# AnnSeidel/genometools

Measured on AMD Instinct MI355X. Metric: Gbp/s ESA build (suf+lcp+bwt), 3 Gbp DNA, 1/2/4/8 MI355X; bit-exact vs CPU, higher is better.
Workload: dtype u64; 1 GPU; human-like DNA (2% N, 24 seqs, repeats) n=3000000000 seed=43 -suf -lcp -bwt (BASELINE.json configs[2]); parallelism=1 device, pair_suffixes=341032298, tied_suffixes=390540711, refine_rounds=9, maxbranchdepth=8256

## Files before the change

genometools_amd/_lib.py:

```python
import ctypes
import os
import subprocess

HERE = os.path.dirname(os.path.abspath(__file__))
ROOT = os.path.dirname(HERE)
LIB_PATH = os.path.join(HERE, "libgtamd_esa.so")
SOURCES = [os.path.join(HERE, "csrc", f) for f in
           ("esa_prims.hip", "esa_engine.hip", "esa_synth.hip", "esa_encode.hip",
            "esa_pck.hip", "esa_comm.hip")]
HEADERS = [os.path.join(HERE, "csrc", f) for f in ("esa_common.h", "esa_prims.h", "esa_devutil.h", "esa_msd.h", "esa_msd_blocks.h",
                                                     "esa_pck_replay.h")] + \
          [os.path.join(ROOT, "include", h) for h in ("gtamd_esa.h", "gtamd_encode.h", "gtamd_pck.h")]
HIPCC = os.environ.get("HIPCC", "/opt/rocm/bin/hipcc")


def needs_build():
    if not os.path.exists(LIB_PATH):
        return True
    t = os.path.getmtime(LIB_PATH)
    return any(os.path.getmtime(p) > t for p in SOURCES + HEADERS)


def build_library(force=False, verbose=False):
    if not force and not needs_build():
        return LIB_PATH
    cmd = [HIPCC, "--offload-arch=gfx950", "-O3", "-std=c++17", "-fPIC",
           "-shared", "-Wall", "-Wno-unused-function", "-o", LIB_PATH] + SOURCES
    if verbose:
        print(" ".join(cmd))
    subprocess.run(cmd, check=True)
    return LIB_PATH


class EsaStats(ctypes.Structure):
    _fields_ = [("totallength", ctypes.c_uint64),
                ("numberofallsortedsuffixes", ctypes.c_uint64),
                ("longest", ctypes.c_uint64),
                ("largelcpvalues", ctypes.c_uint64),
                ("maxbranchdepth", ctypes.c_uint64),
                ("lcptabsum", ctypes.c_uint64),
                ("prefixlength", ctypes.c_uint32),
                ("refine_rounds", ctypes.c_uint32),
                ("tied_suffixes", ctypes.c_uint64),
                ("pair_suffixes", ctypes.c_uint64),
                ("device_bytes", ctypes.c_uint64),
                ("msd_big_entries", ctypes.c_uint64),
                ("msd_crowded_entries", ctypes.c_uint64),
                ("rank_entries_built", ctypes.c_uint64)]


class EsaTiming(ctypes.Structure):
    _fields_ = [("total_ms", ctypes.c_float),
                ("keygen_ms", ctypes.c_float),
                ("sort_ms", ctypes.c_float),
                ("finalize_ms", ctypes.c_float),
                ("refine_ms", ctypes.c_float),
                ("tie_fix_ms", ctypes.c_float),
                ("scatter_ms", ctypes.c_float),
                ("scatter_launches", ctypes.c_uint32),
                ("scatter_items", ctypes.c_uint64),
                ("comm_ms", ctypes.c_float),
                ("comm_calls", ctypes.c_uint32),
                ("comm_bytes", ctypes.c_uint64),
                ("alloc_ms", ctypes.c_float),
                ("dominant_kernel", ctypes.c_uint32),
                ("scatter_read_items", ctypes.c_uint64),
                ("scatter_written_items", ctypes.c_uint64)]


class EncodeSummary(ctypes.Structure):
    _fields_ = [(name, ctypes.c_uint64) for name in
                ("totallength", "numofsequences", "specialcharacters",
                 "realspecialranges")] + \
               [("specialrangestab", ctypes.c_uint64 * 3)] + \
               [(name, ctypes.c_uint64) for name in
                ("lengthofspecialprefix", "lengthofspecialsuffix", "wildcards",
                 "realwildcardranges")] + \
               [("wildcardrangestab", ctypes.c_uint64 * 3)] + \
               [(name, ctypes.c_uint64) for name in
                ("lengthofwildcardprefix", "lengthofwildcardsuffix",
                 "lengthoflongestnonspecial", "minseqlen", "maxseqlen",
                 "equallength")] + \
               [("characterdistribution", ctypes.c_uint64 * 32),
                ("originaldistribution", ctypes.c_uint64 * 256)]


class PckParams(ctypes.Structure):
    _fields_ = [("block_size", ctypes.c_uint32), ("bucket_blocks", ctypes.c_uint32),
                ("locate_interval", ctypes.c_uint32), ("feature_toggles", ctypes.c_int32),
                ("with_statistics", ctypes.c_int32)]


class PckInfo(ctypes.Structure):
    _fields_ = [(name, ctypes.c_uint64) for name in
                ("file_bytes", "cw_data_pos", "var_data_pos", "range_enc_pos",
                 "num_buckets", "num_regions", "var_bits")] + \
               [("cw_bits", ctypes.c_uint32), ("build_ms", ctypes.c_float)]


_P = ctypes.c_void_p
_U64 = ctypes.c_uint64
_U32 = ctypes.c_uint32
_INT = ctypes.c_int
ABI = {
    "gtamd_device_count": (_INT, []),
    "gtamd_esa_last_error": (ctypes.c_char_p, []),
    "gtamd_recommended_prefixlength": (_U32, [_U32, _U64]),
    "gtamd_abi_selftest": (_INT, [_U64]),
    "gtamd_esa_create": (_P, [_INT, _U64, _U32]),
    "gtamd_esa_destroy": (None, [_P]),
    "gtamd_esa_set_part": (_INT, [_P, _U32, _U32]),
    "gtamd_esa_set_prefixlength": (_INT, [_P, _U32]),
    "gtamd_esa_set_readmode": (_INT, [_P, _INT]),
    "gtamd_esa_set_comm": (_INT, [_P, _P, _P, _P]),
    "gtamd_comm_threads_create": (_P, [_U32]),
    "gtamd_comm_rccl_unique_id": (_INT, [_P]),
    "gtamd_comm_rccl_create": (_P, [_P, _U32, _U32, _INT]),
    "gtamd_comm_attach": (_INT, [_P, _U32, _P, _INT]),
    "gtamd_comm_abort": (None, [_P]),
    "gtamd_esa_set_comm_abort": (_INT, [_P, _P, _P]),
    "gtamd_comm_destroy": (None, [_P]),
    "gtamd_esa_set_sequence_bytes": (_INT, [_P, _P, _U64, _INT]),
    "gtamd_esa_set_sequence_packed": (_INT, [_P, _P, _P, _U64]),
    "gtamd_esa_run": (_INT, [_P, _U32]),
    "gtamd_esa_table_entries": (_U64, [_P, _INT]),
    "gtamd_esa_table_offset": (_U64, [_P]),
    "gtamd_esa_bck_layout": (_INT, [_P, ctypes.POINTER(_U64), ctypes.POINTER(_U64),
                                    ctypes.POINTER(_U64)]),
    "gtamd_esa_table_device": (_P, [_P, _INT]),
    "gtamd_esa_table_copy": (_INT, [_P, _INT, _P, _U64, _U64]),
    "gtamd_esa_get_stats": (_INT, [_P, ctypes.POINTER(EsaStats)]),
# ... 77 lines not shown
```

genometools_amd/csrc/esa_engine.hip:

```cpp
#include <stdarg.h>
#include <stdlib.h>
#include <chrono>
#include <type_traits>
#include <utility>
#include <vector>
#include "../../include/gtamd_esa.h"
#include "esa_prims.h"
#include "esa_devutil.h"

static thread_local char g_err[1024] = "";
void gtamd_set_error(const char *fmt, ...) {
  va_list ap;
  va_start(ap, fmt);
  vsnprintf(g_err, sizeof g_err, fmt, ap);
  va_end(ap);
}
extern "C" const char *gtamd_esa_last_error(void) { return g_err; }

extern "C" int gtamd_device_count(void) {
  GTAMD_ABI_BEGIN
  int n = 0;
  if (hipGetDeviceCount(&n) != hipSuccess) return 0;
  return n;
  GTAMD_ABI_END(0)
// ... 1927 lines not shown
        const u32 e = e0 + c;
        if ((startflags >> c) & 1u) {
          const bool open = RK::open(s_key[e]);
          if (e < cnt && !open) {
            const u32 size = (u32) s_start[lgw + 1] - e;
            gmax = size > gmax ? size : gmax;
          }
          lgw--;
        }
      }
    }
#pragma unroll
    for (int d = 32; d >= 1; d >>= 1) {
      const u32 o = __shfl_xor(gmax, d, 64);
      gmax = o > gmax ? o : gmax;
    }
    if ((tid & 63) == 0) s_scan[tid >> 6] = gmax;
    __syncthreads();
    gmax = s_scan[0];
    for (int i = 1; i < RT_THREADS / 64; i++) gmax = s_scan[i] > gmax ? s_scan[i] : gmax;
    __syncthreads();
    if (gmax <= 32u) {
      for (u32 ph = 0; ph <= gmax; ph++) {
        const u32 odd = ph & 1u;
#pragma unroll
        for (int c = 0; c < RT_PER / 2; c++) {
          const u32 lo = 2u * ((u32) c * RT_THREADS + tid) + odd;
          if (lo + 1 < (u32) RT_TILE) {
            const u64 a = s_key[lo], b = s_key[lo + 1];
            if (a > b) { s_key[lo] = b; s_key[lo + 1] = a; }
          }
        }
        __syncthreads();
      }
    } else {
      for (u32 k = 2; k <= (u32) RT_TILE; k <<= 1) {
        for (u32 j = k >> 1; j > 0; j >>= 1) {
#pragma unroll
          for (int c = 0; c < RT_PER / 2; c++) {
            const u32 idx = (u32) c * RT_THREADS + tid;
            const u32 lo = ((idx & ~(j - 1)) << 1) | (idx & (j - 1));
            const u32 hi = lo + j;
            const bool up = (lo & k) == 0;
            const u64 a = s_key[lo], b = s_key[hi];
            if ((a > b) == up) { s_key[lo] = b; s_key[hi] = a; }
          }
          __syncthreads();
        }
      }
    }
  }
  u32 hval[RT_PER], hmax = 0;
#pragma unroll
  for (int c = 0; c < RT_PER; c++) {
    const u32 e = e0 + c;
    const u64 key = s_key[e];
    const bool head = e == 0 || (key >> 11) != (s_key[e - 1] >> 11);
    const u32 v = (head && e < cnt) ? uidx[base + e] : 0u;
    hval[c] = v;
    hmax = v > hmax ? v : hmax;
  }
  u32 carry = block_scan_excl_max(hmax, &tot, s_scan);
#pragma unroll
  for (int c = 0; c < RT_PER; c++) {
    const u32 e = e0 + c;
    carry = hval[c] > carry ? hval[c] : carry;
    if (e < cnt) {
      const u64 key = s_key[e];
      const u32 src = (u32) (key & 2047u);
      if (!RK::open(key)) {
        cv[base + e] = s_pos[src];
        hv[base + e] = carry;
      }
    }
  }
  (void) nflag;
  __syncthreads();
  }
}

constexpr int RT_STRIDE_MIN = 512;
__global__ __launch_bounds__(256) void k_tile_starts(const u32 *__restrict__ ugrp, u64 m,
                                                     u32 ntiles, u32 stride,
                                                     u32 *__restrict__ tstart) {
  const u32 t = blockIdx.x * 256 + threadIdx.x;
  if (t > ntiles) return;
  if (t == ntiles) { tstart[t] = (u32) m; return; }
  const u64 s = (u64) t * stride;
  const u32 g = ugrp[s];
  u64 lo = s > (u64) RT_TILE ? s - RT_TILE : 0, hi = s;
  if (ugrp[lo] == g) {
    tstart[t] = (u32) (lo == 0 ? 0 : s);
    return;
  }
  while (hi - lo > 1) {
    const u64 mid = (lo + hi) >> 1;
    if (ugrp[mid] == g) hi = mid; else lo = mid;
  }
  tstart[t] = (u32) hi;
}

__global__ __launch_bounds__(256) void k_flag_count(const u32 *__restrict__ flagbits, u64 m,
                                                    u32 nblocks, u32 *__restrict__ blkcnt) {
  const u32 b = blockIdx.x * 256 + threadIdx.x;
  if (b >= nblocks) return;
  u32 c = 0;
  for (int w = 0; w < RT_TILE / 32; w++) c += (u32) __popc(flagbits[(u64) b * (RT_TILE / 32) + w]);
  blkcnt[b] = c;
  (void) m;
}

template <typename P>
__global__ __launch_bounds__(RT_THREADS) void k_flag_gather(
    const u32 *__restrict__ flagbits, const u32 *__restrict__ tileoff,
    const u32 *__restrict__ ugrp, const P *__restrict__ k2,
    const P *__restrict__ upos, u64 m, P *__restrict__ fk2, P *__restrict__ fk2_sort,
    u32 *__restrict__ fgrp, P *__restrict__ fpos, u32 *__restrict__ fj,
    u32 *__restrict__ perm) {
  __shared__ u32 s_scan[4];
  const u64 base = (u64) blockIdx.x * RT_TILE + (u64) threadIdx.x * RT_PER;
  const u32 f = base < m ? (u32) reinterpret_cast<const u8 *>(flagbits)[(u64) blockIdx.x * RT_THREADS + threadIdx.x] : 0u;
  const u32 cnt = (u32) __popc(f);
  u32 tot;
  u32 o = tileoff[blockIdx.x] + block_scan_excl_sum(cnt, &tot, s_scan);
  if (f == 0) return;
#pragma unroll
  for (int c = 0; c < RT_PER; c++)
    if ((f >> c) & 1u) {
      const u64 j = base + c;
      const P k = k2[j];
      fk2[o] = k;
      fk2_sort[o] = k;
      fgrp[o] = ugrp[j];
      fpos[o] = upos[j];
      fj[o] = (u32) j;
      perm[o] = o;
      o++;
    }
}

__global__ __launch_bounds__(256) void k_gather_u32(const u32 *__restrict__ src,
                                                    const u32 *__restrict__ idx, u64 n,
                                                    u32 *__restrict__ dst) {
  const u64 r = (u64) blockIdx.x * 256 + threadIdx.x;
  if (r < n) dst[r] = src[idx[r]];
}

template <typename P>
__global__ __launch_bounds__(256) void k_flag_heads(
    const u32 *__restrict__ perm, const u32 *__restrict__ fgrp, const P *__restrict__ fk2,
    const P *__restrict__ fpos, const u32 *__restrict__ uidx, const u32 *__restrict__ fj,
    u64 nf, u32 *__restrict__ fhv, P *__restrict__ cvs) {
  const u64 r = (u64) blockIdx.x * 256 + threadIdx.x;
  if (r >= nf) return;
  const u32 a = perm[r];
  bool head = r == 0;
  if (!head) {
    const u32 b = perm[r - 1];
    head = fgrp[a] != fgrp[b] || fk2[a] != fk2[b];
  }
  fhv[r] = head ? uidx[fj[r]] : 0u;
  cvs[r] = fpos[a];
}

template <typename P>
__global__ __launch_bounds__(256) void k_flag_scatter(
    const P *__restrict__ cvs, const u32 *__restrict__ fhv,
    const u32 *__restrict__ fj, u64 nf, P *__restrict__ cv,
    u32 *__restrict__ hv) {
  const u64 r = (u64) blockIdx.x * 256 + threadIdx.x;
  if (r >= nf) return;
  const u32 j = fj[r];
  cv[j] = cvs[r];
  hv[j] = fhv[r];
}

template <typename P>
__global__ __launch_bounds__(256) void k_round_apply(
    const P *__restrict__ cval, const u32 *__restrict__ gnew,
    const u32 *__restrict__ uidx, const u32 *__restrict__ ugrp, u64 m,
    u64 rank_offset, P *__restrict__ sa, P *__restrict__ rank,
    u64 *__restrict__ keep, u32 *__restrict__ blockcnt) {
  __shared__ u32 s_cnt[4];
  const u64 j = (u64) blockIdx.x * 256 + threadIdx.x;
  bool kept = false;
  if (j < m) {
    const P p = cval[j];
    const u32 g = gnew[j], i = uidx[j];
    if (rank != nullptr && g != ugrp[j]) rank[p] = (P) (rank_offset + g);
    const bool head = g == i;
    const bool nexthead = j + 1 == m || gnew[j + 1] == uidx[j + 1];
    const bool resolved = head && nexthead;
    if (resolved) sa[i] = p;
    kept = !resolved;
  }
  const u64 b = __ballot(kept);
  if ((threadIdx.x & 63) == 0) {
    keep[((u64) blockIdx.x * 256 + threadIdx.x) >> 6] = b;
    s_cnt[threadIdx.x >> 6] = (u32) __popcll(b);
  }
  __syncthreads();
  if (threadIdx.x == 0) blockcnt[blockIdx.x] = s_cnt[0] + s_cnt[1] + s_cnt[2] + s_cnt[3];
}

template <typename P>
__global__ __launch_bounds__(256) void k_round_compact(
    const u64 *__restrict__ keep, const u32 *__restrict__ boff,
    const u32 *__restrict__ blockcnt, const u32 *__restrict__ uidx,
    const P *__restrict__ cval, const u32 *__restrict__ gnew, u64 m,
    u32 *__restrict__ uidx2, P *__restrict__ upos2, u32 *__restrict__ ugrp2,
    Stats *stats) {
  __shared__ u32 s_scan[4];
  const u64 j = (u64) blockIdx.x * 256 + threadIdx.x;
  const u32 k = (u32) (keep[j >> 6] >> (j & 63)) & 1u;
  u32 tot;
  const u32 o = boff[blockIdx.x] + block_scan_excl_sum(k, &tot, s_scan);
  if (k) {
    uidx2[o] = uidx[j];
    upos2[o] = cval[j];
    ugrp2[o] = gnew[j];
  }
  if (blockIdx.x == gridDim.x - 1 && threadIdx.x == 0)
    stats->count = boff[blockIdx.x] + blockcnt[blockIdx.x];
}

__global__ void k_total(const u32 *__restrict__ off, const u32 *__restrict__ cnt,
                        u64 n, Stats *stats) {
  stats->count = n ? off[n - 1] + cnt[n - 1] : 0u;
}

__global__ void k_total2(const u32 *__restrict__ off, const u32 *__restrict__ cnt,
                         u64 n, Stats *stats) {
  stats->count2 = n ? off[n - 1] + cnt[n - 1] : 0u;
}
__global__ void k_total3(const u32 *__restrict__ off, const u32 *__restrict__ cnt,
                         u64 n, Stats *stats) {
  stats->count3 = n ? off[n - 1] + cnt[n - 1] : 0u;
}

constexpr int DIRECT_MAX_GROUP = 16;
constexpr u64 DIRECT_MAX_LCP = 250;

template <int BITS>
__device__ bool suffix_less(const Text &t, u64 p, u64 q, bool *deep) {
  const u64 l = lcp_extend<BITS>(t, p, q, (u64) Key<BITS>::KNOWN, DIRECT_MAX_LCP);
  if (l >= DIRECT_MAX_LCP) { *deep = true; return p < q; }
  const bool sp = is_special(t, p + l), sq = is_special(t, q + l);
  if (sp || sq) return (sp && sq) ? p < q : sq;
  return Sym<BITS>::at(t, p + l) < Sym<BITS>::at(t, q + l);
}

template <int BITS, typename P>
__global__ __launch_bounds__(256) void k_direct_ties(
    Text t, const u32 *__restrict__ uidx0, const u32 *__restrict__ ugrp, u64 m0,
    P *__restrict__ sa, u64 *__restrict__ suf, u8 *__restrict__ lcp,
    u8 *__restrict__ bwt, bool want_lcp, u64 index_offset, Stats *stats) {
  const u64 j = (u64) blockIdx.x * 256 + threadIdx.x;
// ... 1113 lines not shown
  gtamd_set_error("slice of %llu entries exceeds the 32-bit index range of one "
                  "part: use more parts", (unsigned long long) NL);
}

struct WinFilterTies {
  const u64 *tiebits2;
  const u32 *carry;
  const u64 *swp;
};
template <typename Q>
static int launch_win_filter(gtamd_esa_ctx *c, const Switches &sw, const Q *sa, u64 NL, int wb,
                             const u32 *sel, u64 nww, u32 nww_global, const u32 *pref,
                             const WinFilterTies &t, Q *fpos, u32 *fhead, u64 cap, u64 windows) {
  hipStream_t st = c->st;
  const bool wf_lds = (nww + 4) * 5 <= WF_LDS_MAX && !sw.win_filter_global;
  if (sw.debug)
    fprintf(stderr, "gtamd: part %u: win filter: bitmap=%s windows=%llu\n", c->part,
            wf_lds ? "lds" : "global", (unsigned long long) windows);
  const u32 grid = (u32) div_up(NL, WF_SPAN * WF_ITER);
  if (wf_lds) {
    HIP_TRY(hipFuncSetAttribute(reinterpret_cast<const void *>(&k_win_filter<Q, true>),
                                hipFuncAttributeMaxDynamicSharedMemorySize,
                                (int) wf_lds_bytes<Q>(nww, true)));
    k_win_filter<Q, true><<<grid, WF_THREADS, wf_lds_bytes<Q>(nww, true), st>>>(
        sa, NL, wb, sel, (u32) nww, pref, t.tiebits2, t.carry, t.swp, fpos, fhead, cap, c->d_stats);
  } else
    k_win_filter<Q, false><<<grid, WF_THREADS, wf_lds_bytes<Q>(0, false), st>>>(
        sa, NL, wb, sel, nww_global, pref, t.tiebits2, t.carry, t.swp, fpos, fhead, cap, c->d_stats);
  HIP_TRY(hipGetLastError());
  return 0;
}

template <int BITS, bool WIDE>
struct Build {
  using K = Key<BITS>;
  using P = typename std::conditional<WIDE, u64, u32>::type;
  static constexpr u64 RANKREC = 1 + sizeof(P) / 4;
  static constexpr u64 ISA_CHUNK = 1ull << 27;

  gtamd_esa_ctx *const c;
  const Switches &sw;
  u32 want;
  const bool dist;
  const u64 N, n;
  const u32 R;
  const hipStream_t st;
  const bool debug;

  u32 prefixlength = 0;
  bool long_prefix = false, want_suf = false, want_lcp = false, want_bwt = false;
  bool msd = false;
  bool msd_part = false;
  bool fused_pass0 = false;

  int fail = 0;

  u64 NL, index_offset = 0;
  Tiles tl;
  u64 Tn;
  u64 prev_key = 0;
  int has_prev = 0;

  bool pass0_done = false;
  u32 *msd_sa = nullptr, *msd_fval = nullptr;
  u64 *msd_fkey = nullptr, msd_local = 0;
  int nev = 0;
  u64 *skey = nullptr;
  P *sa = nullptr;
  u64 *fkey = nullptr;
  u32 *fval = nullptr;
  u64 *d_suf = nullptr;
  u8 *d_lcp = nullptr, *d_bwt = nullptr;
  bool emitted = false;

  u64 *tiebits = nullptr;
  u64 *tiebits2 = nullptr;
  u64 numties = 0, anyties = 0;
  u64 nwords = 0, nwb = 0;
  u64 m0 = 0;
  u64 m0_tied_all = 0;
  u64 anyleft = 0;
  u64 npairs = 0, nsmall = 0, nrec = 0;
  u64 rank_built = 0;
  u32 rounds = 0;
  int nb = 0, nbl = 0;
  int ps[8], pw[8], pn = 0;

  struct Words {
    u32 *cntw, *headw, *offw, *carry;
    u32 *pcnt, *poff;
    u32 *scnt, *soff;
    u32 *rcnt, *roff;
    u32 *scanws;
    u32 *pws;
    void carve(u32 *base, u64 nw) {
      cntw = base;
      headw = cntw + nw + 16;
      offw = headw + nw + 16;
      carry = offw + nw + 16;
      pcnt = carry + nw + 16;
      poff = pcnt + nw + 16;
      scnt = poff + nw + 16;
      soff = scnt + nw + 16;
      rcnt = soff + nw + 16;
      roff = rcnt + nw + 16;
      scanws = roff + nw + 16;
      pws = scanws + scan_workspace_words(nw) + 64;
    }
  } wd;

  struct PairLists {
    P *pk_a, *pk_b;
    u64 *pv_a, *pv_b;
    u32 *pidx, *pres, *prws, *sidx, *sres, *slcp, *srec;
    u8 *ssize;
    u64 *swp;
    void carve(Bump &a, u64 records, u64 pairs, u64 groups, u64 nw) {
      const u64 pp = (records + 64 + 3) & ~3ull;
      const u64 sp = (groups + 64 + 3) & ~3ull;
      pk_a = a.take<P>(pp); pk_b = a.take<P>(pp);
      pv_a = a.take<u64>(pp); pv_b = a.take<u64>(pp);
      pidx = a.take<u32>(pp); pres = a.take<u32>(pp);
      prws = a.take<u32>(radix_workspace_words(records));
      sidx = a.take<u32>(sp); sres = a.take<u32>(sp); slcp = a.take<u32>(3 * sp);
      srec = a.take<u32>(sp);
      ssize = a.take<u8>(sp);
      swp = a.take<u64>(pairs > 0 ? 2 * nw + 8 : 0);
    }
  } pl;
  const u64 *pair_swp = nullptr;
  int apply_early = 0;
  u64 apply_wgs = 256;
  u32 *lcpfull = nullptr;

  struct Rounds {
    u32 *uidx0, *uidx, *ugrp, *uidx2, *ugrp2;
    P *upos, *upos2;
    P *cvo;
    u32 *hv;
    u64 *keep;
    u32 *koff;
    P *k2;
    u32 *flagbits;
    u32 *tstart;
    P *fk2, *fk2s_a, *fk2s_b, *fpos, *cvs;
    u32 *fgrp, *fj, *perm_a, *perm_b, *gk_a, *gk_b, *fhv;
    P *lk_a, *lk_b;
    u32 *lv_a, *lv_b;
    u32 *rws2, *scanws2;
    u32 *xoff, *xorder, *xqoff, *xmsg, *xbc_q, *xbo_q, *xbc_u, *xbo_u;
    P *xrank, *xans;
    u8 *xdest_q, *xdest_u;
    void carve(Bump &a, u64 mp, u64 tied, u64 items, u32 parts, bool exchange) {
      uidx0 = a.take<u32>(mp); uidx = a.take<u32>(mp); ugrp = a.take<u32>(mp);
      uidx2 = a.take<u32>(mp); ugrp2 = a.take<u32>(mp);
      upos = a.take<P>(mp); upos2 = a.take<P>(mp);
      cvo = a.take<P>(mp);
      hv = a.take<u32>(mp);
      keep = a.take<u64>(mp / 64 + 4);
      koff = a.take<u32>(mp);
      k2 = a.take<P>(mp);
      flagbits = a.take<u32>(mp / 32 + RT_TILE / 32 + 64);
      tstart = a.take<u32>(mp / RT_STRIDE_MIN + 64);
      fk2 = a.take<P>(mp); fk2s_a = a.take<P>(mp); fk2s_b = a.take<P>(mp);
      fpos = a.take<P>(mp); cvs = a.take<P>(mp);
      fgrp = a.take<u32>(mp); fj = a.take<u32>(mp);
// ... 1014 lines not shown
    }
    if (more) {
      TRY(send_ranks());
      TRY(dest_count(c, s.rq, m, ar.xdest_q, ar.xbc_q, ar.xbo_q, ar.scanws2, 0));
    }
    if (s.m_upd > 0) TRY(dest_place(c, s.ru, s.m_upd, ar.xdest_u, ar.xbo_u));
    s.m_upd = 0;
    s.rq.sendq = ar.xqoff; s.rq.order = ar.xorder;
    TRY(dest_place(c, s.rq, m, ar.xdest_q, ar.xbo_q));
    if (R == 1) {
      if (m > 0) {
        k_local_lookups<P><<<(u32) div_up(m, 256), 256, 0, st>>>(s.rq, m);
        HIP_TRY(hipGetLastError());
      }
      return 0;
    }
    constexpr u32 W = (u32) RANKREC;
    FuseTab ts, tr;
    ts.n = tr.n = R;
    std::vector<u64> sendw(R), recvw(R), sq(R), rqc(R);
    ts.upre[0] = ts.qpre[0] = tr.upre[0] = tr.qpre[0] = 0;
    ts.wpre[0] = tr.wpre[0] = 0;
    for (u32 r = 0; r < R; r++) {
      const u64 us = mine[R + r], qs = mine[r];
      const u64 ur = gathered[(size_t) r * GW + R + c->part], qr = gathered[(size_t) r * GW + c->part];
      sendw[r] = us * W + qs; recvw[r] = ur * W + qr;
      sq[r] = qs; rqc[r] = qr;
      ts.upre[r + 1] = ts.upre[r] + (u32) us; ts.qpre[r + 1] = ts.qpre[r] + (u32) qs;
      ts.wpre[r + 1] = ts.wpre[r] + sendw[r];
      tr.upre[r + 1] = tr.upre[r] + (u32) ur; tr.qpre[r + 1] = tr.qpre[r] + (u32) qr;
      tr.wpre[r + 1] = tr.wpre[r] + recvw[r];
    }
    const u32 parts = R;
    const bool toobig =
        tile_overrun([&gathered, GW, parts](u32 p, u32 q) { return gathered[(size_t) p * GW + parts + q]; }) ||
        tile_overrun([&gathered, GW](u32 p, u32 q) { return gathered[(size_t) p * GW + q]; });
    if (toobig || (u64) tr.upre[R] + 64 > xrecv_n || (u64) tr.qpre[R] + 64 > xrecv_n) {
      gtamd_set_error("rank exchange: %u updates and %u queries for a tile of %llu positions",
                      tr.upre[R], tr.qpre[R], (unsigned long long) Tn);
      return -1;
    }
    const u64 nsend = (u64) ts.upre[R] + ts.qpre[R];
    if (nsend > 0) {
      k_fuse_pack<P><<<(u32) div_up(nsend, 256), 256, 0, st>>>(ts, ar.xoff, ar.xrank, ar.xqoff, ar.xmsg);
      HIP_TRY(hipGetLastError());
    }
    TRY(comm_alltoallv(c, ar.xmsg, sendw.data(), xrecv_msg, recvw.data(), 4, "new ranks and queries"));
    if (tr.upre[R] > 0) {
      k_fuse_updates<P><<<(u32) div_up(tr.upre[R], 256), 256, 0, st>>>(tr, xrecv_msg, isa);
      HIP_TRY(hipGetLastError());
    }
    if (tr.qpre[R] > 0) {
      k_fuse_answers<P><<<(u32) div_up(tr.qpre[R], 256), 256, 0, st>>>(tr, xrecv_msg, isa, xrecv_ans);
      HIP_TRY(hipGetLastError());
    }
    if (m > 0) {
      k_local_lookups<P><<<(u32) div_up(m, 256), 256, 0, st>>>(s.rq, m);
      HIP_TRY(hipGetLastError());
    }
    TRY(comm_alltoallv(c, xrecv_ans, rqc.data(), ar.xans, sq.data(), sizeof(P), "answers"));
    if (ts.qpre[R] > 0) {
      k_k2_scatter<P><<<(u32) div_up(ts.qpre[R], 256), 256, 0, st>>>(ar.xans, ar.xorder, ts.qpre[R], ar.k2);
      HIP_TRY(hipGetLastError());
    }
    return 0;
  }

  int refine_round(RoundState &s) {
    const u64 m = s.m, h = s.h;
    if (!dist && rk.windows && h > rk.h0) {
      HIP_TRY(hipMemsetAsync(&c->d_stats->count2, 0, 4, st));
      k_win_check<P><<<(u32) div_up(m, 256), 256, 0, st>>>(ar.upos, m, h, rk.wb, rk.nwin, rk.w_built,
                                                         rk.w_need, c->d_stats);
      HIP_TRY(hipGetLastError());
      TRY(fetch_stats(c));
      if (c->h_stats->count2 != 0) TRY(build_rank(false));
    }
    const u32 rt_stride = sw.round_stride;
    const u32 g = (u32) div_up(m, 256);
    const u32 ntiles = (u32) div_up(m, rt_stride);
    const u32 nfb = (u32) div_up(m, RT_TILE);
    u32 *tilecnt = ar.koff, *tileoff = ar.koff + nfb + 16;
    HIP_TRY(hipMemsetAsync(ar.flagbits, 0, (u64) nfb * (RT_TILE / 8), st));
    k_tile_starts<<<ntiles / 256 + 1, 256, 0, st>>>(ar.ugrp, m, ntiles, rt_stride, ar.tstart);
    HIP_TRY(hipGetLastError());
    k_round_tile<P><<<ntiles, RT_THREADS, 0, st>>>(
        ar.uidx, ar.upos, ar.ugrp, ar.k2, m, ar.cvo, ar.hv, ar.tstart, ar.flagbits, dist ? nullptr : rank, h, n);
    HIP_TRY(hipGetLastError());
    k_flag_count<<<nfb / 256 + 1, 256, 0, st>>>(ar.flagbits, m, nfb, tilecnt);
    HIP_TRY(hipGetLastError());
    TRY(scan_u32(SCAN_SUM, tilecnt, tileoff, nfb, false, ar.scanws2, st));
    k_total<<<1, 1, 0, st>>>(tileoff, tilecnt, nfb, c->d_stats);
    HIP_TRY(hipGetLastError());
    TRY(fetch_stats(c));
    const u64 nf = c->h_stats->count;
    if (debug)
      fprintf(stderr, "gtamd: part %u round %u: %llu entries in groups across tile borders "
              "(%u tiles, stride %u)\n", c->part, rounds, (unsigned long long) nf, ntiles, rt_stride);
    if (nf > 0) {
      k_flag_gather<P><<<nfb, RT_THREADS, 0, st>>>(ar.flagbits, tileoff, ar.ugrp, ar.k2, ar.upos, m, ar.fk2,
                                                     ar.fk2s_a, ar.fgrp, ar.fpos, ar.fj, ar.perm_a);
      HIP_TRY(hipGetLastError());
      TRY(radix_sort_pairs<P, u32>(ar.fk2s_a, ar.perm_a, ar.fk2s_b, ar.perm_b, nf, ps, pw, pn, ar.rws2, st,
                                   nullptr, nullptr));
      u32 *perm1 = (pn & 1) ? ar.perm_b : ar.perm_a, *permx = (pn & 1) ? ar.perm_a : ar.perm_b;
      const u32 gf = (u32) div_up(nf, 256);
      k_gather_u32<<<gf, 256, 0, st>>>(ar.fgrp, perm1, nf, ar.gk_a);
      HIP_TRY(hipGetLastError());
      TRY(radix_sort_pairs<u32, u32>(ar.gk_a, perm1, ar.gk_b, permx, nf, s.gs, s.gw, s.gn, ar.rws2, st,
                                     nullptr, nullptr));
      const u32 *perm2 = (s.gn & 1) ? permx : perm1;
      k_flag_heads<P><<<gf, 256, 0, st>>>(perm2, ar.fgrp, ar.fk2, ar.fpos, ar.uidx, ar.fj, nf, ar.fhv, ar.cvs);
      HIP_TRY(hipGetLastError());
      TRY(scan_u32(SCAN_MAX, ar.fhv, ar.fhv, nf, true, ar.scanws2, st));
      k_flag_scatter<P><<<gf, 256, 0, st>>>(ar.cvs, ar.fhv, ar.fj, nf, ar.cvo, ar.hv);
      HIP_TRY(hipGetLastError());
    }
    u32 *bcnt = ar.koff, *boffs = ar.koff + g + 16;
    k_round_apply<P><<<g, 256, 0, st>>>(ar.cvo, ar.hv, ar.uidx, ar.ugrp, m, index_offset, sa,
                                        dist ? nullptr : rank, ar.keep, bcnt);
    HIP_TRY(hipGetLastError());
    TRY(scan_u32(SCAN_SUM, bcnt, boffs, g, false, ar.scanws2, st));
    k_round_compact<P><<<g, 256, 0, st>>>(ar.keep, boffs, bcnt, ar.uidx, ar.cvo, ar.hv, m, ar.uidx2,
                                          ar.upos2, ar.ugrp2, c->d_stats);
    HIP_TRY(hipGetLastError());
    TRY(fetch_stats(c));
    s.m = c->h_stats->count;
    s.h *= 2;
    if (dist) {
      s.ru.cval = ar.cvo; s.ru.gnew = ar.hv; s.ru.ugrp = ar.ugrp; s.ru.index_offset = index_offset;
      s.ru.tl = tl; s.ru.isa = isa; s.ru.soff = ar.xoff; s.ru.srank = ar.xrank;
      s.m_upd = m;
      TRY(dest_count(c, s.ru, s.m_upd, ar.xdest_u, ar.xbc_u, ar.xbo_u, ar.scanws2, 1));
      s.rq.upos = ar.upos2; s.rq.h = s.h;
      TRY(dest_count(c, s.rq, s.m, ar.xdest_q, ar.xbc_q, ar.xbo_q, ar.scanws2, 0));
    }
    std::swap(ar.uidx, ar.uidx2);
    std::swap(ar.ugrp, ar.ugrp2);
    std::swap(ar.upos, ar.upos2);
    if (dist) s.ru.ugrp = ar.ugrp2;
    return 0;
  }

  int tie_fix() {
    TRY(launch_emission());
    HIP_TRY(hipStreamWaitEvent(st, c->ev_emitted, 0));
    if (want_lcp && !apply_early) {
      if (!dist) lcpfull = fval;
      else if (WIDE) lcpfull = fval;
      else lcpfull = c->isa_tmp.as<u32>();
    }
    if (!apply_early) TRY(launch_apply(st));
    const u32 g0 = (u32) div_up(m0, 256);
    u32 *bcnt0 = ar.koff, *boff0 = ar.koff + g0 + 16;
    if (m0 > 0) {
      TRY(fork_second_stream());
      k_fix_basic<BITS, P><<<g0, 256, 0, c->st2>>>(c->text, ar.uidx0, m0, sa, d_suf, d_bwt,
                                                   c->d_stats, index_offset);
      HIP_TRY(hipGetLastError());
      HIP_TRY(hipEventRecord(c->ev_emitted, c->st2));
    }
    if (want_lcp && m0 > 0) {
      k_tied_counts<<<g0, 256, 0, st>>>(ar.uidx0, m0, tiebits2, bcnt0);
      HIP_TRY(hipGetLastError());
      TRY(scan_u32(SCAN_SUM, bcnt0, boff0, g0, false, ar.scanws2, st));
      k_total<<<1, 1, 0, st>>>(boff0, bcnt0, g0, c->d_stats);
      HIP_TRY(hipGetLastError());
      TRY(fetch_stats(c));
      const u64 m1 = c->h_stats->count;
      k_lcp_pairs<P><<<g0, 256, 0, st>>>(boff0, tiebits2, ar.uidx0, sa, m0, ar.lk_a, ar.lv_a);
      HIP_TRY(hipGetLastError());
      TRY(radix_sort_pairs<P, u32>(ar.lk_a, ar.lv_a, ar.lk_b, ar.lv_b, m1, ps, pw, pn, ar.rws2, st,
                                   nullptr, nullptr));
      const P *pk = (pn & 1) ? ar.lk_b : ar.lk_a;
      const u32 *pv = (pn & 1) ? ar.lv_b : ar.lv_a;
      k_lcp_chunks<BITS, P><<<stride_grid(div_up(div_up(m1, LCP_CHUNK), 256)), 256, 0, st>>>(
          c->text, pk, pv, m1, sa, d_lcp, lcpfull, c->d_stats);
      HIP_TRY(hipGetLastError());
    }
    if (apply_early) HIP_TRY(hipStreamWaitEvent(st, c->ev_applied, 0));
    if (!want_lcp) return 0;
    TRY(fetch_stats(c));
    const u64 pairs = c->h_stats->numlarge;
    if (pairs > c->llv_cap) {
      free_dev(c->llv);
      c->llv = nullptr;
      c->llv_cap = 0;
      HIP_TRY(hipMalloc(&c->llv, (pairs + pairs / 4 + 1024) * 16));
      c->llv_cap = pairs + pairs / 4 + 1024;
    }
    if (pairs > 0) {
      const u32 gl = (u32) div_up(NL, LLV_TILE);
      u32 *lc = wd.cntw, *lo = wd.offw;
      k_large_counts<<<gl, 256, 0, st>>>(d_lcp, NL, lc);
      HIP_TRY(hipGetLastError());
      TRY(scan_u32(SCAN_SUM, lc, lo, gl, false, wd.scanws, st));
      k_llv_emit<<<gl, 256, 0, st>>>(d_lcp, NL, lcpfull, lo, index_offset, c->llv);
      HIP_TRY(hipGetLastError());
    }
    c->llv_pairs = pairs;
    return 0;
  }

  int report() {
    TRY(launch_emission());
    HIP_TRY(hipStreamWaitEvent(st, c->ev_emitted, 0));
    HIP_TRY(hipEventRecord(c->ev[EV_DONE], st));
    TRY(fetch_stats(c));

    c->stats.totallength = n;
    c->stats.numberofallsortedsuffixes = N;
    c->stats.longest = c->h_stats->longest;
    c->stats.largelcpvalues = want_lcp ? c->h_stats->numlarge : 0;
    c->stats.maxbranchdepth =
        want_lcp ? (c->h_stats->maxlcp > c->h_stats->dmax ? c->h_stats->maxlcp
                                                           : c->h_stats->dmax) : 0;
    c->stats.lcptabsum = want_lcp ? c->h_stats->lcpsum + c->h_stats->dsum : 0;
    if (long_prefix && want_lcp) {
      HIP_TRY(hipMemsetAsync(&c->d_stats->msum, 0, 8, st));
      if (c->NL > 0) {
        k_masked_lcpsum<<<stride_grid(div_up(c->NL, 256)), 256, 0, st>>>(
            c->text, c->suf.as<u64>(), c->lcp.as<u8>(), c->NL, prefixlength, c->d_stats);
        HIP_TRY(hipGetLastError());
      }
      if (c->llv_pairs > 0) {
        k_masked_llvsum<<<stride_grid(div_up(c->llv_pairs, 256)), 256, 0, st>>>(
            c->text, c->suf.as<u64>(), c->llv, c->llv_pairs, c->index_offset, prefixlength,
            c->d_stats);
        HIP_TRY(hipGetLastError());
      }
      TRY(fetch_stats(c));
      c->stats.lcptabsum = c->h_stats->msum;
    }
    c->stats.prefixlength = prefixlength;
    c->stats.refine_rounds = rounds;
    c->stats.tied_suffixes = (m0_tied_all ? m0_tied_all : m0) + 2 * npairs + c->h_stats->smalldone;
    c->stats.pair_suffixes = 2 * npairs;
    c->stats.device_bytes = c->alloc_bytes;
    float ms = 0;
    HIP_TRY(hipEventElapsedTime(&ms, c->ev[EV_START], c->ev[EV_DONE])); c->timing.total_ms = ms;
    HIP_TRY(hipEventElapsedTime(&ms, c->ev[EV_START], c->ev[EV_KEYS])); c->timing.keygen_ms = ms;
    HIP_TRY(hipEventElapsedTime(&ms, c->ev[EV_KEYS], c->ev[EV_SORTED])); c->timing.sort_ms = ms;
    HIP_TRY(hipEventElapsedTime(&ms, c->ev[EV_SORTED], c->ev[EV_TIEBITS])); c->timing.finalize_ms = ms;
    HIP_TRY(hipEventElapsedTime(&ms, c->ev[EV_REFINE_BEGIN], c->ev[EV_REFINE_END])); c->timing.refine_ms = ms;
    HIP_TRY(hipEventElapsedTime(&ms, c->ev[EV_REFINE_END], c->ev[EV_DONE])); c->timing.tie_fix_ms = ms;
    float sc = 0;
    for (int i = 0; i < nev; i++) {
      HIP_TRY(hipEventElapsedTime(&ms, c->ev_scatter[2 * i], c->ev_scatter[2 * i + 1]));
      sc += ms;
    }
    if (msd && msd_local > 0) {
      HIP_TRY(hipEventElapsedTime(&sc, c->ev_scatter[0], c->ev_scatter[1]));
      nev = 1;
    }
    c->timing.scatter_ms = sc;
    c->timing.scatter_launches = (u32) nev;
    c->timing.scatter_items = msd ? msd_local : NL;
    c->timing.scatter_read_items = c->timing.scatter_items;
    c->timing.scatter_written_items = msd ? msd_local - c->h_stats->crowded : NL;
    c->stats.msd_crowded_entries = msd ? c->h_stats->crowded : 0;
    c->stats.rank_entries_built = rank_built;
    c->timing.dominant_kernel = msd ? 1u : 0u;
    c->timing.alloc_ms = c->alloc_ms;
    c->want = want;
    c->ran = true;
    return 0;
  }
};

extern "C" int gtamd_esa_run(gtamd_esa_ctx *c, uint32_t want) {
  GTAMD_ABI_BEGIN
  if (c == nullptr) { gtamd_set_error("null context"); return -1; }
  struct AbortOnFailure {
    gtamd_esa_ctx *c;
    bool ok;
    ~AbortOnFailure() {
      if (!ok && c->numparts > 1 && c->comm_abort != nullptr) c->comm_abort(c->comm_abort_user);
    }
  } guard = {c, false};
  if (!c->have_text) { gtamd_set_error("no sequence set"); return -1; }
  if ((want & 15u) == 0) { gtamd_set_error("nothing requested"); return -1; }
  HIP_TRY(hipSetDevice(c->device));
  const Switches sw = read_switches();
  if (sw.debug)
    fprintf(stderr, "gtamd: part %u: switches: msd=%d msd_part_off=%d msd_cbits=%d msd_big_max=%u "
            "msd_radix=%d msd_pack=%d msd_pack_cap=%u msd_bin_limit=%u fused_pass0=%d "
            "force_wide=%d no_pairs=%d no_small_groups=%d apply_early=%d apply_wgs=%llu "
            "apply_wgs_given=%d rank_window_bits=%d rank_all_windows=%d win_filter_global=%d "
            "pair_chunk=%d round_stride=%u debug=%d\n",
            c->part, sw.msd, (int) sw.msd_part_off, sw.msd_cbits, sw.msd_big_max, (int) sw.msd_radix,
            (int) sw.msd_pack, sw.msd_pack_cap, sw.msd_bin_limit, (int) sw.fused_pass0,
            (int) sw.force_wide, (int) sw.no_pairs, (int) sw.no_small_groups, sw.apply_early,
            (unsigned long long) sw.apply_wgs, (int) sw.apply_wgs_given, sw.rank_window_bits,
            (int) sw.rank_all_windows, (int) sw.win_filter_global, sw.pair_chunk, sw.round_stride,
            (int) sw.debug);
  const bool wide = sw.force_wide || c->N >= SINGLE_LIMIT;
  const bool dist = c->numparts > 1 || wide;
  if (c->numparts == 1 && c->N >= SINGLE_LIMIT) {
    gtamd_set_error("sequence of %llu symbols exceeds the 32-bit index range of a "
                    "single build: build it in parts (gtamd_esa_set_part)",
                    (unsigned long long) c->n);
    return -1;
  }
  int rc;
  if (c->bits == 2)
    rc = wide ? Build<2, true>(c, sw, want, dist).run() : Build<2, false>(c, sw, want, dist).run();
  else
    rc = wide ? Build<5, true>(c, sw, want, dist).run() : Build<5, false>(c, sw, want, dist).run();
  guard.ok = rc == 0;
  return rc;
  GTAMD_ABI_END(-1)
}

extern "C" uint64_t gtamd_esa_table_entries(const gtamd_esa_ctx *c,
                                            gtamd_table which) {
  GTAMD_ABI_BEGIN
  if (c == nullptr || !c->ran) return 0;
  if (which == GTAMD_TAB_BCK)
    return (c->want & GTAMD_WANT_BCK) ? c->bck_codes + 1 + c->bck_special + c->bck_dist : 0;
  return which == GTAMD_TAB_LLV ? c->llv_pairs : c->NL;
  GTAMD_ABI_END(0)
}
extern "C" int gtamd_esa_bck_layout(const gtamd_esa_ctx *c, uint64_t *numofallcodes,
                                    uint64_t *numofspecialcodes,
                                    uint64_t *numofdistpfxidxcounters) {
  GTAMD_ABI_BEGIN
  if (c == nullptr || !c->ran || !(c->want & GTAMD_WANT_BCK)) {
    gtamd_set_error("no bucket table was requested");
    return -1;
  }
  *numofallcodes = c->bck_codes;
  *numofspecialcodes = c->bck_special;
  *numofdistpfxidxcounters = c->bck_dist;
  return 0;
  GTAMD_ABI_END(-1)
}
extern "C" uint64_t gtamd_esa_table_offset(const gtamd_esa_ctx *c) {
  GTAMD_ABI_BEGIN
  return (c == nullptr || !c->ran) ? 0 : c->index_offset;
  GTAMD_ABI_END(0)
}
extern "C" const void *gtamd_esa_table_device(const gtamd_esa_ctx *c,
                                              gtamd_table which) {
  GTAMD_ABI_BEGIN
// ... 90 lines not shown
```

include/gtamd_esa.h:

```cpp
#ifndef GTAMD_ESA_H
#define GTAMD_ESA_H

#include <stddef.h>
#include <stdint.h>

#ifdef __cplusplus
extern "C" {
#endif

#define GTAMD_WILDCARD   254u
#define GTAMD_SEPARATOR  255u
#define GTAMD_UNDEFBWT   254u
#define GTAMD_LCPOVERFLOW 255u

#define GTAMD_WANT_SUF 1u
#define GTAMD_WANT_LCP 2u
#define GTAMD_WANT_BWT 4u
#define GTAMD_WANT_BCK 8u

typedef enum {
  GTAMD_TAB_SUF = 0,
  GTAMD_TAB_LCP = 1,
  GTAMD_TAB_BWT = 2,
  GTAMD_TAB_LLV = 3,
  GTAMD_TAB_BCK = 4
} gtamd_table;

typedef struct {
  uint64_t totallength;
  uint64_t numberofallsortedsuffixes;
  uint64_t longest;
  uint64_t largelcpvalues;
  uint64_t maxbranchdepth;
  uint64_t lcptabsum;
  uint32_t prefixlength;
  uint32_t refine_rounds;
  uint64_t tied_suffixes;
  uint64_t pair_suffixes;
  uint64_t device_bytes;
  uint64_t msd_big_entries;
  uint64_t msd_crowded_entries;
  uint64_t rank_entries_built;
} gtamd_esa_stats;

typedef struct {
  float total_ms;
  float keygen_ms;
  float sort_ms;
  float finalize_ms;
  float refine_ms;
  float tie_fix_ms;
  float scatter_ms;
  uint32_t scatter_launches;
  uint64_t scatter_items;
  float comm_ms;
  uint32_t comm_calls;
  uint64_t comm_bytes;
  float alloc_ms;
  uint32_t dominant_kernel;
  uint64_t scatter_read_items;
  uint64_t scatter_written_items;
} gtamd_esa_timing;

typedef struct gtamd_esa_ctx gtamd_esa_ctx;

int gtamd_device_count(void);
const char *gtamd_esa_last_error(void);

uint32_t gtamd_recommended_prefixlength(uint32_t numofchars, uint64_t n);
int gtamd_abi_selftest(uint64_t host_bytes);

gtamd_esa_ctx *gtamd_esa_create(int device, uint64_t max_n,
                                uint32_t numofchars);
void gtamd_esa_destroy(gtamd_esa_ctx *ctx);

int gtamd_esa_set_part(gtamd_esa_ctx *ctx, uint32_t part, uint32_t numparts);

typedef int (*gtamd_allgather_fn)(void *user, const void *send, void *recv,
                                  uint32_t bytes);
typedef int (*gtamd_alltoallv_fn)(void *user, const void *send,
                                  const uint64_t *sendcounts, void *recv,
                                  const uint64_t *recvcounts,
                                  uint32_t elem_bytes, void *stream);
int gtamd_esa_set_comm(gtamd_esa_ctx *ctx, gtamd_allgather_fn allgather,
                       gtamd_alltoallv_fn alltoallv, void *user);
int gtamd_esa_set_comm_abort(gtamd_esa_ctx *ctx, void (*abort_fn)(void *user), void *user);

typedef struct gtamd_comm gtamd_comm;
gtamd_comm *gtamd_comm_threads_create(uint32_t numparts);
int gtamd_comm_rccl_unique_id(uint8_t id[128]);
gtamd_comm *gtamd_comm_rccl_create(const uint8_t id[128], uint32_t rank,
                                   uint32_t numparts, int device);
int gtamd_comm_attach(gtamd_comm *comm, uint32_t part, gtamd_esa_ctx *ctx,
                      int device);
void gtamd_comm_abort(gtamd_comm *comm);
void gtamd_comm_destroy(gtamd_comm *comm);

int gtamd_esa_set_readmode(gtamd_esa_ctx *ctx, int readmode);

int gtamd_esa_set_prefixlength(gtamd_esa_ctx *ctx, uint32_t prefixlength);

int gtamd_esa_set_sequence_bytes(gtamd_esa_ctx *ctx, const uint8_t *enc,
                                 uint64_t n, int is_device);

int gtamd_esa_set_sequence_packed(gtamd_esa_ctx *ctx, const uint64_t *twobit,
                                  const uint64_t *specialbits, uint64_t n);

int gtamd_esa_run(gtamd_esa_ctx *ctx, uint32_t want);

uint64_t gtamd_esa_table_entries(const gtamd_esa_ctx *ctx, gtamd_table which);
uint64_t gtamd_esa_table_offset(const gtamd_esa_ctx *ctx);
int gtamd_esa_bck_layout(const gtamd_esa_ctx *ctx, uint64_t *numofallcodes,
                         uint64_t *numofspecialcodes,
                         uint64_t *numofdistpfxidxcounters);
const void *gtamd_esa_table_device(const gtamd_esa_ctx *ctx, gtamd_table which);
int gtamd_esa_table_copy(gtamd_esa_ctx *ctx, gtamd_table which, void *dst,
                         uint64_t first, uint64_t count);
int gtamd_esa_get_stats(const gtamd_esa_ctx *ctx, gtamd_esa_stats *st);
int gtamd_esa_get_timing(const gtamd_esa_ctx *ctx, gtamd_esa_timing *tm);

int gtamd_esa_build(const uint8_t *enc, uint64_t n, uint32_t numofchars,
                    uint32_t want, uint64_t *suf, uint8_t *lcp, uint8_t *bwt,
                    uint64_t *llv, uint64_t llv_capacity, uint64_t *llv_pairs,
                    gtamd_esa_stats *st);

// ... 8 lines not shown
```

Before: 25.85 Gbp/s.

## Sort tile-crossing rank groups in LDS with a block-local radix kernel

Groups that straddle round-tile borders are now listed by a new kernel. Groups up to about 30K entries are handled by a 1024-thread workgroup that radix-sorts indices by k2 digits in shared memory and writes cv/hv directly. Only larger groups still take the global flag-gather/sort path, and k_flag_count plus the scan are skipped when no such group exists. This replaces global sorting of cross-tile entries with per-group LDS work, at the cost of an extra list kernel, atomics and large LDS use per block.

```diff
diff --git a/genometools_amd/_lib.py b/genometools_amd/_lib.py
--- a/genometools_amd/_lib.py
+++ b/genometools_amd/_lib.py
@@ -46,7 +46,8 @@
                 ("device_bytes", ctypes.c_uint64),
                 ("msd_big_entries", ctypes.c_uint64),
                 ("msd_crowded_entries", ctypes.c_uint64),
-                ("rank_entries_built", ctypes.c_uint64)]
+                ("rank_entries_built", ctypes.c_uint64),
+                ("round_lds_entries", ctypes.c_uint64)]
 
 
 class EsaTiming(ctypes.Structure):
diff --git a/genometools_amd/csrc/esa_engine.hip b/genometools_amd/csrc/esa_engine.hip
--- a/genometools_amd/csrc/esa_engine.hip
+++ b/genometools_amd/csrc/esa_engine.hip
@@ -2033,10 +2033,14 @@
 constexpr int RT_STRIDE_MIN = 512;
 __global__ __launch_bounds__(256) void k_tile_starts(const u32 *__restrict__ ugrp, u64 m,
                                                      u32 ntiles, u32 stride,
-                                                     u32 *__restrict__ tstart) {
+                                                     u32 *__restrict__ tstart, Stats *stats) {
   const u32 t = blockIdx.x * 256 + threadIdx.x;
   if (t > ntiles) return;
-  if (t == ntiles) { tstart[t] = (u32) m; return; }
+  if (t == ntiles) {
+    tstart[t] = (u32) m;
+    stats->count = stats->count2 = stats->count3 = 0;
+    return;
+  }
   const u64 s = (u64) t * stride;
   const u32 g = ugrp[s];
   u64 lo = s > (u64) RT_TILE ? s - RT_TILE : 0, hi = s;
@@ -2124,6 +2128,173 @@
   const u32 j = fj[r];
   cv[j] = cvs[r];
   hv[j] = fhv[r];
+}
+
+constexpr int RC_THREADS = 1024;
+constexpr int RC_PER = 30;
+constexpr int RC_CAP = RC_THREADS * RC_PER;
+constexpr int RC_DIGITS = 16;
+constexpr u32 RC_LDS_BYTES = (2u * RC_CAP + (u32) RC_DIGITS * RC_THREADS) * 2u;
+
+__global__ __launch_bounds__(256) void k_cross_list(const u32 *__restrict__ flagbits,
+                                                    const u32 *__restrict__ ugrp, u64 m,
+                                                    u32 nwords, u32 *__restrict__ gfirst,
+                                                    u32 *__restrict__ glen, Stats *stats) {
+  const u32 w = blockIdx.x * 256 + threadIdx.x;
+  const u32 f = w < nwords ? flagbits[w] : 0u;
+  u32 np = (u32) __popc(f);
+#pragma unroll
+  for (int d = 32; d >= 1; d >>= 1) np += __shfl_xor(np, d, 64);
+  if ((threadIdx.x & 63) == 0 && np != 0) atomicAdd(&stats->count, np);
+  if (f == 0) return;
+  const u64 base = (u64) w * 32;
+  u32 gprev = base > 0 ? ugrp[base - 1] : 0u;
+  u32 g[32];
+#pragma unroll
+  for (int b = 0; b < 32; b++) g[b] = base + b < m ? ugrp[base + b] : 0xFFFFFFFFu;
+  u32 starts = 0;
+#pragma unroll
+  for (int b = 0; b < 32; b++) {
+    if (((f >> b) & 1u) && (base + b == 0 || g[b] != gprev)) starts |= 1u << b;
+    gprev = g[b];
+  }
+  while (starts != 0) {
+    const u64 j = base + (u32) (__ffs((int) starts) - 1);
+    starts &= starts - 1;
+    const u32 gj = ugrp[j];
+    u64 lo = j, hi = j + RC_CAP;
+    if (hi >= m) hi = m;
+    else if (ugrp[hi] == gj) { lo = hi; hi = m; }
+    const bool over = lo != j;
+    while (hi - lo > 1) {
+      const u64 mid = (lo + hi) >> 1;
+      if (ugrp[mid] == gj) lo = mid; else hi = mid;
+    }
+    const u32 len = (u32) (hi - j);
+    if (over) atomicAdd(&stats->count3, len);
+    else {
+      const u32 o = atomicAdd(&stats->count2, 1u);
+      gfirst[o] = (u32) j;
+      glen[o] = len;
+    }
+  }
+}
+
+template <typename P>
+__global__ __launch_bounds__(RC_THREADS) __attribute__((amdgpu_waves_per_eu(5))) void k_round_cross(
+    const u32 *__restrict__ gfirst, const u32 *__restrict__ glen,
+    const u32 *__restrict__ uidx, const P *__restrict__ upos, const P *__restrict__ k2,
+    P *__restrict__ cv, u32 *__restrict__ hv, u32 *__restrict__ clearbits) {
+  extern __shared__ u16 rc_lds[];
+  __shared__ u32 s_scan[RC_THREADS / 64];
+  __shared__ u32 s_diff[2];
+  u16 *cur = rc_lds, *nxt = rc_lds + RC_CAP, *cnt = rc_lds + 2 * RC_CAP;
+  const u32 tid = threadIdx.x;
+  const u32 first = gfirst[blockIdx.x], len = glen[blockIdx.x];
+  const u32 per = (len + RC_THREADS - 1) / RC_THREADS;
+  const u32 e0 = tid * per;
+  const u32 mine = e0 >= len ? 0u : (len - e0 < per ? len - e0 : per);
+  if (tid < 2) s_diff[tid] = 0;
+  if (clearbits != nullptr) {
+    const u32 end = first + len;
+    for (u32 w = (first >> 5) + tid; w <= ((end - 1) >> 5); w += RC_THREADS) {
+      const u32 a = w * 32 > first ? 0u : first & 31u;
+      const u32 b = w * 32 + 32 <= end ? 32u : end & 31u;
+      const u32 mask = (b == 32u ? ~0u : (1u << b) - 1u) & ~((1u << a) - 1u);
+      atomicAnd(&clearbits[w], ~mask);
+    }
+  }
+  __syncthreads();
+  constexpr int RC_STEP = 10;
+  {
+    const u64 kfirst = (u64) k2[first];
+    u64 d = 0;
+    for (u32 c0 = 0; c0 < mine; c0 += RC_STEP) {
+#pragma unroll
+      for (int c = 0; c < RC_STEP; c++)
+        if (c0 + c < mine) {
+          cur[e0 + c0 + c] = (u16) (e0 + c0 + c);
+          d |= (u64) k2[first + e0 + c0 + c] ^ kfirst;
+        }
+    }
+    if ((u32) d != 0) atomicOr(&s_diff[0], (u32) d);
+    if ((u32) (d >> 32) != 0) atomicOr(&s_diff[1], (u32) (d >> 32));
+  }
+  __syncthreads();
+  const u64 diff = (u64) s_diff[0] | ((u64) s_diff[1] << 32);
+  for (int p = 0; p < (int) sizeof(P) * 2; p++) {
+    if (((diff >> (4 * p)) & 15ull) == 0) continue;
+    u32 v[RC_PER];
+#pragma unroll
+    for (int c = 0; c < RC_PER; c++) v[c] = cur[(u32) c < mine ? e0 + c : len - 1];
+#pragma unroll
+    for (int c = 0; c < RC_PER; c++)
+      v[c] |= ((u32) ((u64) k2[first + v[c]] >> (4 * p)) & 15u) << 16;
+#pragma unroll
+    for (int d = 0; d < RC_DIGITS; d++) cnt[d * RC_THREADS + tid] = 0;
+#pragma unroll
+    for (int c = 0; c < RC_PER; c++)
+      if ((u32) c < mine) cnt[(v[c] >> 16) * RC_THREADS + tid] += 1;
+    __syncthreads();
+    {
+      u32 x[RC_DIGITS], sum = 0;
+#pragma unroll
+      for (int i = 0; i < RC_DIGITS; i++) { x[i] = cnt[tid * RC_DIGITS + i]; sum += x[i]; }
+      u32 tot;
+      u32 o = block_scan_excl<SCAN_SUM, RC_THREADS>(sum, &tot, s_scan);
+#pragma unroll
+      for (int i = 0; i < RC_DIGITS; i++) { cnt[tid * RC_DIGITS + i] = (u16) o; o += x[i]; }
+    }
+    __syncthreads();
+#pragma unroll
+    for (int c = 0; c < RC_PER; c++)
+      if ((u32) c < mine) {
+        const u32 ci = (v[c] >> 16) * RC_THREADS + tid;
+        const u32 o = cnt[ci];
+        cnt[ci] = (u16) (o + 1);
+        nxt[o] = (u16) v[c];
+      }
+    __syncthreads();
+    u16 *t = cur; cur = nxt; nxt = t;
+  }
+  u32 heads = 0, hmax = 0;
+  u64 kprev = (mine > 0 && e0 > 0) ? (u64) k2[first + cur[e0 - 1]] : 0ull;
+  for (u32 c0 = 0; c0 < mine; c0 += RC_STEP) {
+    u64 kv[RC_STEP];
+#pragma unroll
+    for (int c = 0; c < RC_STEP; c++)
+      kv[c] = c0 + c < mine ? (u64) k2[first + cur[e0 + c0 + c]] : 0ull;
+    u32 hd = 0;
+#pragma unroll
+    for (int c = 0; c < RC_STEP; c++) {
+      if (c0 + c < mine && (e0 + c0 + c == 0 || kv[c] != kprev)) hd |= 1u << c;
+      kprev = kv[c];
+    }
+    u32 uv[RC_STEP];
+#pragma unroll
+    for (int c = 0; c < RC_STEP; c++) uv[c] = ((hd >> c) & 1u) ? uidx[first + e0 + c0 + c] : 0u;
+#pragma unroll
+    for (int c = 0; c < RC_STEP; c++) hmax = uv[c] > hmax ? uv[c] : hmax;
+    heads |= hd << c0;
+  }
+  u32 tot;
+  u32 carry = block_scan_excl<SCAN_MAX, RC_THREADS>(hmax, &tot, s_scan);
+  for (u32 c0 = 0; c0 < mine; c0 += RC_STEP) {
+    u32 uv[RC_STEP];
+    P pv[RC_STEP];
+#pragma unroll
+    for (int c = 0; c < RC_STEP; c++) {
+      uv[c] = ((heads >> (c0 + c)) & 1u) ? uidx[first + e0 + c0 + c] : 0u;
+      pv[c] = c0 + c < mine ? upos[first + cur[e0 + c0 + c]] : (P) 0;
+    }
+#pragma unroll
+    for (int c = 0; c < RC_STEP; c++)
+      if (c0 + c < mine) {
+        carry = uv[c] > carry ? uv[c] : carry;
+        cv[first + e0 + c0 + c] = pv[c];
+        hv[first + e0 + c0 + c] = carry;
+      }
+  }
 }
 
 template <typename P>
@@ -3403,6 +3574,8 @@
   u64 anyleft = 0;
   u64 npairs = 0, nsmall = 0, nrec = 0;
   u64 rank_built = 0;
+  u64 round_lds = 0;
+  bool cross_lds_set = false;
   u32 rounds = 0;
   int nb = 0, nbl = 0;
   int ps[8], pw[8], pn = 0;
@@ -4583,21 +4756,38 @@
     const u32 nfb = (u32) div_up(m, RT_TILE);
     u32 *tilecnt = ar.koff, *tileoff = ar.koff + nfb + 16;
     HIP_TRY(hipMemsetAsync(ar.flagbits, 0, (u64) nfb * (RT_TILE / 8), st));
-    k_tile_starts<<<ntiles / 256 + 1, 256, 0, st>>>(ar.ugrp, m, ntiles, rt_stride, ar.tstart);
+    k_tile_starts<<<ntiles / 256 + 1, 256, 0, st>>>(ar.ugrp, m, ntiles, rt_stride, ar.tstart, c->d_stats);
     HIP_TRY(hipGetLastError());
     k_round_tile<P><<<ntiles, RT_THREADS, 0, st>>>(
         ar.uidx, ar.upos, ar.ugrp, ar.k2, m, ar.cvo, ar.hv, ar.tstart, ar.flagbits, dist ? nullptr : rank, h, n);
     HIP_TRY(hipGetLastError());
-    k_flag_count<<<nfb / 256 + 1, 256, 0, st>>>(ar.flagbits, m, nfb, tilecnt);
-    HIP_TRY(hipGetLastError());
-    TRY(scan_u32(SCAN_SUM, tilecnt, tileoff, nfb, false, ar.scanws2, st));
-    k_total<<<1, 1, 0, st>>>(tileoff, tilecnt, nfb, c->d_stats);
+    u32 *gfirst = ar.fj, *glen = ar.fgrp;
+    const u32 nfw = nfb * (RT_TILE / 32);
+    k_cross_list<<<nfw / 256 + 1, 256, 0, st>>>(ar.flagbits, ar.ugrp, m, nfw, gfirst, glen, c->d_stats);
     HIP_TRY(hipGetLastError());
     TRY(fetch_stats(c));
-    const u64 nf = c->h_stats->count;
+    const u64 nall = c->h_stats->count;
+    const u32 ngroups = c->h_stats->count2;
+    const u64 nf = c->h_stats->count3;
     if (debug)
       fprintf(stderr, "gtamd: part %u round %u: %llu entries in groups across tile borders "
-              "(%u tiles, stride %u)\n", c->part, rounds, (unsigned long long) nf, ntiles, rt_stride);
+              "(%u tiles, stride %u)\n", c->part, rounds, (unsigned long long) nall, ntiles, rt_stride);
+    if (ngroups > 0) {
+      if (!cross_lds_set) {
+        HIP_TRY(hipFuncSetAttribute(reinterpret_cast<const void *>(&k_round_cross<P>),
+                                    hipFuncAttributeMaxDynamicSharedMemorySize, (int) RC_LDS_BYTES));
+        cross_lds_set = true;
+      }
+      k_round_cross<P><<<ngroups, RC_THREADS, RC_LDS_BYTES, st>>>(gfirst, glen, ar.uidx, ar.upos, ar.k2, ar.cvo,
+                                                                   ar.hv, nf > 0 ? ar.flagbits : nullptr);
+      HIP_TRY(hipGetLastError());
+      round_lds += nall - nf;
+    }
+    if (nf > 0) {
+      k_flag_count<<<nfb / 256 + 1, 256, 0, st>>>(ar.flagbits, m, nfb, tilecnt);
+      HIP_TRY(hipGetLastError());
+      TRY(scan_u32(SCAN_SUM, tilecnt, tileoff, nfb, false, ar.scanws2, st));
+    }
     if (nf > 0) {
       k_flag_gather<P><<<nfb, RT_THREADS, 0, st>>>(ar.flagbits, tileoff, ar.ugrp, ar.k2, ar.upos, m, ar.fk2,
                                                      ar.fk2s_a, ar.fgrp, ar.fpos, ar.fj, ar.perm_a);
@@ -4761,6 +4951,7 @@
     c->timing.scatter_written_items = msd ? msd_local - c->h_stats->crowded : NL;
     c->stats.msd_crowded_entries = msd ? c->h_stats->crowded : 0;
     c->stats.rank_entries_built = rank_built;
+    c->stats.round_lds_entries = round_lds;
     c->timing.dominant_kernel = msd ? 1u : 0u;
     c->timing.alloc_ms = c->alloc_ms;
     c->want = want;
diff --git a/include/gtamd_esa.h b/include/gtamd_esa.h
--- a/include/gtamd_esa.h
+++ b/include/gtamd_esa.h
@@ -41,6 +41,7 @@
   uint64_t msd_big_entries;
   uint64_t msd_crowded_entries;
   uint64_t rank_entries_built;
+  uint64_t round_lds_entries;
 } gtamd_esa_stats;
 
 typedef struct {
```

Result: no change. 25.80 Gbp/s (-0.2%).
